# NVlabs/neuralrgbd

Measured on AMD Instinct MI355X. Metric: depth frames/sec @256x192x64cand, 5-view window; warp-kernel HBM GB/s vs peak, higher is better.
Workload: dtype f32; 1 GPU; plane-sweep grid 256x192x64cand (image 1024x768); config_id=B, depth_candidates=64, views=5, streams_per_gpu=1, streams_total=1, parallelism=replicas x1 (independent video streams)

## Files before the change

### include/nrgbd.h

```cpp
#ifndef NRGBD_H
#define NRGBD_H

#ifdef __cplusplus
extern "C" {
#endif

#define NRGBD_OK             0
#define NRGBD_E_NULL        -1
#define NRGBD_E_SHAPE       -2
#define NRGBD_E_ALIGN       -3
#define NRGBD_E_ARG         -4

#define NRGBD_DIST_L2        0
#define NRGBD_DIST_L1        1

#define NRGBD_MAX_D        256
#define NRGBD_MAX_V         16

#define NRGBD_INTERFACE_VERSION "0.10"
const char* nrgbd_version(void);
const char* nrgbd_strerror(int code);

int nrgbd_homography_terms(const float* K, const float* R, long r_view_stride, long r_row_stride,
                           const float* t, long t_view_stride, long t_elem_stride, float* KR, float* Kt,
// ... 130 lines not shown
int nrgbd_conv3d_wgrad_f32(const float* x, const float* gy, float* partial, float* dw,
                           int D, int H, int W, int Cin, void* stream);
int nrgbd_bn3d_finalize(const float* stats, int num_workgroups, long count,
                        const float* gamma, const float* beta, float eps, float momentum,
                        float* running_mean, float* running_var, float* scale_shift, unsigned int* collapse_count, long long* batches_tracked, void* stream);

int nrgbd_bn2d_partial_floats(int C);
int nrgbd_bn2d_train_act(const float* x, const float* gamma, const float* beta, float eps, int act,
                         const float* residual, float* y, float* partial, float* mean_var,
                         int N, int C, long HW, void* stream);
int nrgbd_avgpool8(const float* x, float* y, int NC, int H, int W, void* stream);
int nrgbd_avgpool_cl(const float* x, float* y, int N, int H, int W, int C, int k, void* stream);
int nrgbd_conv2d_few_f32(const float* x, int ldx, const float* w_packed, const float* bias, int out_lrelu, float* y, int ldy,
                         int ycoff, int N, int H, int W, int Cin, int Cout, void* stream);
int nrgbd_scatter_channels(const float* src, long stride_c, long stride_y, long stride_x, int C, int H, int W, float* dst,
                           int ldy, int coff, int n_rep, long rep_stride, void* stream);
int nrgbd_bias_act_nchw(float* x, const float* bias, float slope, int N, int C, long HW, void* stream);

int nrgbd_conv_wino_tiles(int N, int H, int W, int dilation);
int nrgbd_conv_wino_rnet_f32(const float* x, const float* w_wino, const float* bias, int out_lrelu, float* y,
                             int N, int H, int W, int Cin, int Cout, void* stream);
int nrgbd_conv_wino_rnet_ex_f32(const float* x, const float* w_wino, const float* bias, int out_lrelu, float* y,
                                int N, int H, int W, int Cin, int Cout, int ldy, int ycoff, int cout_valid, void* stream);
int nrgbd_conv_wino_pack(const float* w, float* w_wino, int Cin, int Cout, int kd, int transposed, void* stream);
int nrgbd_bn_finalize_cm(const float* stats, int rows, int C, long count, const float* gamma, const float* beta, float eps,
                         float momentum, float* running_mean, float* running_var, float* scale_shift, unsigned int* collapse_count,
                         long long* batches_tracked, void* stream);
int nrgbd_conv_wino_f32(const float* x, const float* x_ss, int x_relu, const float* res, const float* res_ss,
                        int res_relu, float* materialized, const float* w_wino, float* y, float* stats,
                        int N, int H, int W, int Cin, int Cout, int kd, int dilation, void* stream);

int nrgbd_conv_wino_dw_pack(const float* w, float* w_wino, int Cin, int Cout, int transposed, void* stream);
int nrgbd_conv_wino_dw_f32(const float* x, const float* x_ss, int x_relu, const float* res, const float* res_ss,
                           int res_relu, float* materialized, const float* w_wino, float* y, float* stats,
                           int N, int H, int W, int Cin, int Cout, void* stream);
int nrgbd_conv_wino_dw_workgroups(int N, int H, int W, int Cout);
int nrgbd_conv_wino_dw4_pack(const float* w, float* w_wino, int Cin, int Cout, int transposed, void* stream);
int nrgbd_conv_wino_dw4_workspace(int N, int H, int W, int Cout, size_t* bytes);
int nrgbd_conv_wino_dw4_f32(const float* x, const float* x_ss, int x_relu, float x_unit, const float* w_wino, float* y, float* stats,
                            void* workspace, size_t workspace_bytes, int N, int H, int W, int Cin, int Cout, void* stream);
int nrgbd_conv_wino_dw_unit_f32(const float* x, const float* x_ss, float x_unit, const float* w_wino, float* y, float* stats,
                                int N, int H, int W, int Cin, int Cout, void* stream);

int nrgbd_conv2d_rnet_f32(const float* x, const float* w_packed, const float* bias, int out_lrelu, float* y,
                          int ldy, int ycoff, int cout_valid, int mode, int pa, int pb,
                          int N, int H, int W, int Cin, int Cout, void* stream);
// ... 168 lines not shown
```

### neuralrgbd_amd/_lib.py

```python
import ctypes
import os

_HERE = os.path.dirname(os.path.abspath(__file__))
LIB_PATH = os.path.join(_HERE, "csrc", "libnrgbd_hip.so")

_c = ctypes
_P = _c.c_void_p
_F = _c.c_float
_I = _c.c_int
_L = _c.c_long
_D = _c.c_double
_Z = _c.c_size_t

GATHER_MAX_V = 6
DEPTH_MAX_THRESHOLDS = 512
DEPTH_EVAL_MAX_SETS = 8
DGF_TILE = (16, 64)
TSDF_EXTRACT_VOXELS = 1024
TSDF_SCAN_PASS = 1024
TSDF_RAYCAST_MAX_STEPS = 65536
TSDF_RAYCAST_TILE = 16
TSDF_RAYCAST_MAX_SIDE = 16384
ICP_MAX_WG = 256
ICP_RECORD_BYTES = 240
# ... 36 lines not shown
    "nrgbd_logsoftmax_d": (_I, [_P, _P, _F, _P, _I, _L, _P]),
    "nrgbd_depth_regress": (_I, [_P, _P, _P, _P, _I, _L, _P]),
    "nrgbd_export_depth_u16": (_I, [_P, _P, _F, _F, _P, _P, _P, _P, _I, _L, _P]),
    "nrgbd_depth_regress_rows": (_I, [_P, _P, _P, _P, _I, _L, _P]),
    "nrgbd_export_depth_u16_rows": (_I, [_P, _P, _F, _F, _P, _P, _P, _P, _I, _L, _P]),
    "nrgbd_warp_depth_fwd": (_I, [_P, _P, _P, _P, _P, _P, _P, _I, _I, _I, _I, _P]),
    "nrgbd_warp_depth_bwd_workgroups": (_I, [_I, _I]),
    "nrgbd_warp_depth_bwd": (_I, [_P, _P, _P, _P, _P, _P, _P, _P, _P, _P, _I, _I, _I, _I, _P]),
    "nrgbd_lba_pyramid": (_I, [_P, _I, _I, _I, _P, _I, _P, _P]),
    "nrgbd_lba_workgroups": (_I, [_I, _I]),
    "nrgbd_lba_grad": (_I, [_P, _P, _P, _P, _P, _P, _P, _P, _I, _I, _I, _P]),
    "nrgbd_lba_update": (_I, [_P, _I, _P, _P, _P, _I, _I, _I, _I, _I, _I, _I, _D, _I, _I, _P]),
    "nrgbd_conv3d_workgroups": (_I, [_I, _I, _I]),
    "nrgbd_conv3d_pack_weights": (_I, [_P, _P, _I, _P]),
    "nrgbd_conv3d_3x3x3_f32": (_I, [_P, _P, _I, _P, _P, _I, _P, _P, _P, _P, _I, _I, _I, _I, _I, _P]),
    "nrgbd_conv3d_3x3x3_cout1_f32": (_I, [_P, _P, _I, _P, _P, _I, _P, _P, _I, _I, _I, _I, _P]),
    "nrgbd_conv3d_cout1_bwd_workgroups": (_I, [_I, _I, _I, _I]),
    "nrgbd_conv3d_cout1_dgrad_f32": (_I, [_P, _P, _P, _I, _I, _I, _P]),
    "nrgbd_conv3d_cout1_wgrad_workspace": (_I, [_I, _I, _I, _P]),
    "nrgbd_conv3d_cout1_wgrad_f32": (_I, [_P, _P, _P, _P, _Z, _I, _I, _I, _P]),
    "nrgbd_conv_wino_tiles": (_I, [_I, _I, _I, _I]),
    "nrgbd_conv_wino_rnet_f32": (_I, [_P, _P, _P, _I, _P, _I, _I, _I, _I, _I, _P]),
    "nrgbd_conv_wino_rnet_ex_f32": (_I, [_P, _P, _P, _I, _P, _I, _I, _I, _I, _I, _I, _I, _I, _P]),
    "nrgbd_conv_wino_pack": (_I, [_P, _P, _I, _I, _I, _I, _P]),
    "nrgbd_bn_finalize_cm": (_I, [_P, _I, _I, _L, _P, _P, _F, _F, _P, _P, _P, _P, _P, _P]),
    "nrgbd_conv_wino_f32": (_I, [_P, _P, _I, _P, _P, _I, _P, _P, _P, _P, _I, _I, _I, _I, _I, _I, _I, _P]),
    "nrgbd_conv_wino_dw_pack": (_I, [_P, _P, _I, _I, _I, _P]),
    "nrgbd_conv_wino_dw_f32": (_I, [_P, _P, _I, _P, _P, _I, _P, _P, _P, _P, _I, _I, _I, _I, _I, _P]),
    "nrgbd_conv_wino_dw_workgroups": (_I, [_I, _I, _I, _I]),
    "nrgbd_conv_wino_dw_unit_f32": (_I, [_P, _P, _F, _P, _P, _P, _I, _I, _I, _I, _I, _P]),
    "nrgbd_conv_wino_dw4_pack": (_I, [_P, _P, _I, _I, _I, _P]),
    "nrgbd_conv_wino_dw4_workspace": (_I, [_I, _I, _I, _I, _P]),
    "nrgbd_conv_wino_dw4_f32": (_I, [_P, _P, _I, _F, _P, _P, _P, _P, _c.c_size_t, _I, _I, _I, _I, _I, _P]),
    "nrgbd_conv3d_wgrad_workgroups": (_I, []),
    "nrgbd_conv3d_wgrad_ranges": (_I, []),
    "nrgbd_conv3d_wgrad_f32": (_I, [_P, _P, _P, _P, _I, _I, _I, _I, _P]),
    "nrgbd_bn3d_finalize": (_I, [_P, _I, _L, _P, _P, _F, _F, _P, _P, _P, _P, _P, _P]),
    "nrgbd_bn2d_partial_floats": (_I, [_I]),
    "nrgbd_bn2d_train_act": (_I, [_P, _P, _P, _F, _I, _P, _P, _P, _P, _I, _I, _L, _P]),
    "nrgbd_avgpool8": (_I, [_P, _P, _I, _I, _I, _P]),
    "nrgbd_conv2d_few_f32": (_I, [_P, _I, _P, _P, _I, _P, _I, _I, _I, _I, _I, _I, _I, _P]),
    "nrgbd_avgpool_cl": (_I, [_P, _P, _I, _I, _I, _I, _I, _P]),
    "nrgbd_scatter_channels": (_I, [_P, _L, _L, _L, _I, _I, _I, _P, _I, _I, _I, _L, _P]),
    "nrgbd_bias_act_nchw": (_I, [_P, _P, _F, _I, _I, _L, _P]),
    "nrgbd_conv2d_workgroups": (_I, [_I, _I, _I]),
    "nrgbd_conv2d_wgrad_workgroups": (_I, [_I, _I, _I, _I, _I]),
# ... 96 lines not shown
```

### neuralrgbd_amd/csrc/wino_pc.hip

```cpp
#include "wino_pc.hpp"

namespace nrgbd {

namespace {

struct PcLane {
    int kq, jj;
    int msel, cwv;
    int a0, a1;
    unsigned ldy, lane_yoff;
};
template <bool HALF> using PcAcc = f32x4[16][HALF ? 1 : 2];

template <int DIL, int EPI, bool HALF>
__device__ __forceinline__ PcLane pc_lane(const WinoPcArgs& a, int lane, int wv) {
    PcLane c;
    c.kq = lane >> 4; c.jj = lane & 15;
    c.msel = HALF ? (wv >> 1) : 0;
    c.cwv = HALF ? (wv & 1) : wv;
    c.a0 = pc_slot(0, 16 * c.msel + c.jj, c.kq); c.a1 = pc_slot(0, 16 + c.jj, c.kq);
    c.ldy = (EPI == 1 && a.ldy) ? (unsigned)a.ldy : (unsigned)a.Cout;
    c.lane_yoff = (unsigned)c.jj + (unsigned)((DIL * 2 * (c.kq >> 1)) * a.W + 8 * (c.kq & 1) * DIL) * c.ldy;
    return c;
}
// ... 147 lines not shown
    s1 += __shfl_xor(s1, 16, 64); s2 += __shfl_xor(s2, 16, 64);
    s1 += __shfl_xor(s1, 32, 64); s2 += __shfl_xor(s2, 32, 64);
    if (c.kq == 0) {
        const int srow = HALF ? 2 * tl.row + c.msel : tl.row;
        a.stats[(size_t)co * a.rows + srow] = s1;
        a.stats[(size_t)(a.Cout + co) * a.rows + srow] = s2;
    }
}

template <int DIL, int EPI, bool HALF>
__device__ __forceinline__ void pc_epilogue(const PcAcc<HALF>& acc, const WinoPcArgs& a, const PcTile& tl, const PcLane& c) {
    const int co = tl.cg * 64 + c.cwv * 16 + c.jj;
    float* ybase = a.y + (((size_t)tl.n * a.H + tl.y0 + tl.py) * a.W + tl.x0 + tl.px) * c.ldy + (EPI == 1 ? a.ycoff : 0) + tl.cg * 64 + c.cwv * 16;
    const bool cok = EPI != 1 || a.cout_valid == 0 || co < a.cout_valid;
    const bool inside = tl.y0 + tl.py + DIL * (kPcTH - 1) < a.H && tl.x0 + tl.px + DIL * (kPcTW - 1) < a.W;
    float s1 = 0.f, s2 = 0.f;
    float bval = 0.f;
    if constexpr (EPI == 1) bval = a.bias ? a.bias[co] : 0.f;
    if (inside) pc_epilogue_interior<DIL, EPI, HALF>(acc, a, c, ybase, cok, bval, s1, s2);
    else pc_epilogue_edge<DIL, EPI, HALF>(acc, a, tl, c, ybase, cok, bval, s1, s2);
    if (a.stats) pc_store_stats<HALF>(a, tl, c, co, s1, s2);
}

struct PcItems {
    int id0, w4;
    int wr_off[kPcNPF];
    int rdR0, rdR1, rdR2;
    float sg, m1;
    int vslot;
    __device__ __forceinline__ int item_id(int u) const { return id0 + 64 * u; }
    __device__ __forceinline__ int row(int u) const { return (item_id(u) >> 2) / 18; }
    __device__ __forceinline__ int cp(int u) const { const int pi = item_id(u) >> 2; return pi - (pi / 18) * 18; }
    __device__ __forceinline__ int col(int u) const { const int c = cp(u); return c < 9 ? 2 * c : 2 * c - 17; }
};

__device__ __forceinline__ PcItems pc_items(int pw, int lane) {
    PcItems p;
    p.id0 = 192 * pw + lane;
    p.w4 = lane & 3;
#pragma unroll
    for (int u = 0; u < kPcNPF; ++u) {
        const int item = p.item_id(u), e = (item - kPcShItems) >> 2;
        p.wr_off[u] = item < kPcShItems ? (p.row(u) * kPcRawW + p.cp(u)) * kCB + p.w4 * 4
                                        : ((e >> 1) * kPcRawW + 18 + (e & 1)) * kCB + p.w4 * 4;
    }
    const int tword = lane & 3, thalf = (lane >> 4) & 1, txl = ((lane >> 5) << 2) | ((lane >> 2) & 3);
// ... 49 lines not shown
            r.rs[1] = *reinterpret_cast<const f32x4*>(P.ssl + 2 * a.Cin + 2 * (cb * kCB + w4 * 4) + 4);
        }
    }
    const int tz = nx ? P.tn.n : P.tl.n;
    const int z = KD == 3 ? min(max(tz + kd - 1, 0), a.N - 1) : 0;
    const size_t base = ((size_t)z * P.plane + (size_t)(cb * kCB)) * sizeof(float);
    const __amdgpu_buffer_rsrc_t xb = pc_rsrc(reinterpret_cast<const char*>(a.x) + base);
    const __amdgpu_buffer_rsrc_t rb = pc_rsrc(reinterpret_cast<const char*>(RES ? a.res : a.x) + base);
#pragma unroll
    for (int u = 0; u < kPcNPF; ++u) {
        const unsigned o = nx ? P.nxt.off[u] : P.cur.off[u];
        r.pre[u] = pc_bload(xb, o);
        if constexpr (RES) r.prer[u] = pc_bload(rb, o);
    }
}

template <int KD, bool RES, int EPI, bool MAT, bool INTERIOR>
__device__ __forceinline__ void pc_activate_publish(const WinoPcArgs& a, const PcProd& P, const PcRegs<RES>& r, float* raw, int cb, int kd, int z) {
    const f32x2 sc01 = r.ss[0].lo, sh01 = r.ss[0].hi, sc23 = r.ss[1].lo, sh23 = r.ss[1].hi;
    const f32x2 rc01 = r.rs[0].lo, rh01 = r.rs[0].hi, rc23 = r.rs[1].lo, rh23 = r.rs[1].hi;
    const bool wmat = MAT && (KD != 3 || kd == 1) && P.tl.cg == 0;
    constexpr int NU = kPcNPF;
    f32x2 lo[NU], hi[NU];
    if constexpr (EPI == 1) {
#pragma unroll
        for (int i = 0; i < NU; ++i) { lo[i] = r.pre[i].lo; hi[i] = r.pre[i].hi; }
    } else {
#pragma unroll
        for (int i = 0; i < NU; ++i) {
            lo[i] = __builtin_elementwise_fma(r.pre[i].lo, sc01, sh01);
            hi[i] = __builtin_elementwise_fma(r.pre[i].hi, sc23, sh23);
        }
    }
    __builtin_amdgcn_sched_barrier(0);
    if (EPI == 0 && a.x_relu) {
#pragma unroll
        for (int i = 0; i < NU; ++i) { lo[i].x = relu1(lo[i].x); lo[i].y = relu1(lo[i].y); hi[i].x = relu1(hi[i].x); hi[i].y = relu1(hi[i].y); }
    }
    __builtin_amdgcn_sched_barrier(0);
    if constexpr (RES) {
        f32x2 ql[NU], qh[NU];
#pragma unroll
        for (int i = 0; i < NU; ++i) {
            ql[i] = __builtin_elementwise_fma(r.prer[i].lo, rc01, rh01);
            qh[i] = __builtin_elementwise_fma(r.prer[i].hi, rc23, rh23);
        }
        __builtin_amdgcn_sched_barrier(0);
// ... 77 lines not shown
}

template <int KD, int DIL, bool RES, bool ODD = false, int EPI = 0, bool MAT = false, bool HALF = false>
__global__ __launch_bounds__(512) void conv_wino_pc_kernel(const WinoPcArgs a) {
    extern __shared__ __attribute__((aligned(16))) float lds[];
    float* Vb = lds;
    float* rawb = lds + kPcNBuf * kPcV;
    float* ssl = rawb + kPcStrips;

    const int tid = threadIdx.x, lane = tid & 63;
    const int wave = __builtin_amdgcn_readfirstlane(tid >> 6);
    const int wv = wave & 3;
    const int NS = (a.Cin / kCB) * KD;

    int first, step, end;
    pc_tile_share(a.ntiles, first, step, end);
    if (first >= end) return;
    const int count = (end - first + step - 1) / step;
    if constexpr (EPI == 0) {
        pc_load_ss_table<true>(ssl, a.Cin, a.x_ss, RES ? a.res_ss : nullptr, 1.f);
        __syncthreads();
    }

    if (wave >= 4) {
        const PcLane c = pc_lane<DIL, EPI, HALF>(a, lane, wv);
        PcAcc<HALF> acc;
        const f32x4* wbase = reinterpret_cast<const f32x4*>(a.wp) + c.cwv * 64 + lane;
        const size_t wgroup = (size_t)NS * 16 * 256;
        PcTile tl = pc_decode<KD, DIL>(first, a);
        const f32x4* wt = wbase + (size_t)tl.cg * wgroup;
        f32x4 Bn[kPcNB], An[4][2];
        pc_prime_weights<HALF>(Bn, wt);
        __syncthreads();
        __syncthreads();
        __syncthreads();
        pc_prime_a<HALF>(An, Vb, c);
        int buf = 0;
        for (int it = 0; it < count; ++it) {
            const int tnext = first + (it + 1 < count ? it + 1 : it) * step;
            const PcTile tn = pc_decode<KD, DIL>(tnext, a);
            const f32x4* wt_next = wbase + (size_t)tn.cg * wgroup;
            for (int s = 0; s < NS; ++s) {
                const float* Vc = Vb + buf * kPcV;
                const int nbuf = buf == kPcNBuf - 1 ? 0 : buf + 1;
                const float* Vn = Vb + nbuf * kPcV;
                const f32x4* wcur = wt + (size_t)s * (16 * 256);
// ... 86 lines not shown
    }
    const long idx = (long)blockIdx.x * 256 + threadIdx.x;
    if (idx >= total) return;
    long t = idx;
    const int e = t & 3; t >>= 2;
    const int j = t & 15; t >>= 4;
    const int kq = t & 3; t >>= 2;
    const int wave = t & 3; t >>= 2;
    const int xi = t & 15; t >>= 4;
    const int kd = (int)(t % KD); t /= KD;
    const int ncb = Cin / kCB;
    const int cb = (int)(t % ncb);
    const int cg = (int)(t / ncb);
    const int co = cg * 64 + 16 * wave + j, ci = cb * kCB + 4 * kq + e;
    const float* g = transposed ? w + (((size_t)ci * Cout + co) * KD + (KD - 1 - kd)) * 9 : w + (((size_t)co * Cin + ci) * KD + kd) * 9;
    const double G[4][3] = {{1.0, 0.0, 0.0}, {0.5, 0.5, 0.5}, {0.5, -0.5, 0.5}, {0.0, 0.0, 1.0}};
    const int a = xi >> 2, b = xi & 3;
    double u = 0.0;
#pragma unroll
    for (int ky = 0; ky < 3; ++ky)
#pragma unroll
        for (int kx = 0; kx < 3; ++kx) u += G[a][ky] * (double)g[transposed ? (2 - ky) * 3 + (2 - kx) : ky * 3 + kx] * G[b][kx];
    wp[idx] = (float)u;
}

static int pc_workgroups(long ntiles, int* nwg) {
    int dev = 0, ncu = 0;
    hipError_t e = hipGetDevice(&dev);
    if (e == hipSuccess) e = hipDeviceGetAttribute(&ncu, hipDeviceAttributeMultiprocessorCount, dev);
    if (e != hipSuccess) return (int)e;
    if (ncu <= 0) return NRGBD_E_ARG;
    *nwg = ntiles < ncu ? (int)ntiles : ncu;
    return NRGBD_OK;
}

struct PcLaunch { int nwg; size_t lds; int lds_attr; hipStream_t stream; };

template <int KD, int DIL, bool RES, bool ODD = false, int EPI = 0, bool MAT = false, bool HALF = false>
static hipError_t pc_launch(const PcLaunch& L, const WinoPcArgs& a) {
    const hipError_t e = set_max_dynamic_lds(reinterpret_cast<const void*>(&conv_wino_pc_kernel<KD, DIL, RES, ODD, EPI, MAT, HALF>), L.lds_attr);
    if (e != hipSuccess) return e;
    hipLaunchKernelGGL((conv_wino_pc_kernel<KD, DIL, RES, ODD, EPI, MAT, HALF>), dim3(L.nwg), dim3(512), L.lds, L.stream, a);
    return hipSuccess;
}

template <int KD, int DIL, bool HALF>
// ... 83 lines not shown
    if (cout_valid < 0 || cout_valid > Cout || ycoff < 0 || (ldy != 0 && ldy < ycoff + (cout_valid ? cout_valid : Cout))) return NRGBD_E_ARG;
    if ((long)N * H * W * (ldy ? ldy : Cout) >= (1L << 32)) return NRGBD_E_SHAPE;
    const int rows = nrgbd_conv_wino_tiles(N, H, W, 1);
    const long nt = (long)rows * (half ? 1 : Cout / 64);
    if (nt >= (1L << 30)) return NRGBD_E_SHAPE;
    WinoPcArgs a{x, nullptr, nullptr, nullptr, nullptr, w_wino, y, nullptr, 0, 0, N, H, W, Cin, Cout, (int)nt, half ? 2 * rows : rows,
                 bias, out_lrelu, ldy, ycoff, cout_valid};
    int nwg = 0;
    const int rc = pc_workgroups(nt, &nwg);
    if (rc != NRGBD_OK) return rc;
    const size_t lds = (size_t)(kPcNBuf * kPcV + kPcStrips) * sizeof(float);
    const PcLaunch L{nwg, lds, (int)lds, (hipStream_t)stream};
    const bool odd = ((Cin / kCB) & 1) != 0;
    hipError_t e;
    if (odd && half) e = pc_launch<1, 1, false, true, 1, false, true>(L, a);
    else if (odd) e = pc_launch<1, 1, false, true, 1, false, false>(L, a);
    else if (half) e = pc_launch<1, 1, false, false, 1, false, true>(L, a);
    else e = pc_launch<1, 1, false, false, 1, false, false>(L, a);
    if (e != hipSuccess) return (int)e;
    NRGBD_CHECK_LAUNCH();
    return NRGBD_OK;
}

extern "C" int nrgbd_conv_wino_rnet_f32(const float* x, const float* w_wino, const float* bias, int out_lrelu, float* y, int N,
                                        int H, int W, int Cin, int Cout, void* stream) {
    return nrgbd_conv_wino_rnet_ex_f32(x, w_wino, bias, out_lrelu, y, N, H, W, Cin, Cout, 0, 0, 0, stream);
}
```

### neuralrgbd_amd/nets.py

```python
import math

import numpy as np
import torch
import torch.nn as nn
import torch.nn.functional as F


def _conv_bn2d(cin, cout, k, stride, pad, dilation, track=False):
    p = dilation if dilation > 1 else pad
    return nn.Sequential(
        nn.Conv2d(cin, cout, k, stride=stride, padding=p, dilation=dilation, bias=False),
        nn.BatchNorm2d(cout, track_running_stats=track),
    )


def _conv_bn3d(cin, cout):
    return nn.Sequential(nn.Conv3d(cin, cout, 3, stride=1, padding=1, bias=False), nn.BatchNorm3d(cout))


def _conv_lrelu(cin, cout):
    return nn.Sequential(nn.Conv2d(cin, cout, 3, stride=1, padding=1, bias=True), nn.LeakyReLU())


def _deconv_lrelu(cin, cout):
# ... 568 lines not shown
                og = np.ogrid[:n, :n]
                bil = (1 - abs(og[0] - center) / factor) * (1 - abs(og[1] - center) / factor)
                m.weight.data.copy_(torch.from_numpy(bil))

    def _widths(self):
        D = self.conv2_2.out_channels
        C0 = self.conv0[0].in_channels - D
        C1 = self.conv1[0].in_channels - D
        C2 = self.conv2[0].in_channels - D
        ok = 1 <= D <= 128 and (C0, C1, C2) == (64, 32, 3) and self.trans_conv0[0].out_channels == D \
            and self.trans_conv1[0].out_channels == D and self.conv2_1[0].out_channels == D
        return (D, 64 if D <= 64 else 128, C0, C1, C2) if ok else None

    def _levels(self):
        wd = self._widths()
        if wd is not None:
            return ((wd[0], wd[1]),) * 3
        D = self.conv0[0].in_channels - 64
        D0, D1 = self.trans_conv0[0].out_channels, self.conv2_2.out_channels
        ok = D in (32, 64) and (D0, D1) == (2 * D, 4 * D) and self.conv1[0].in_channels == D0 + 32 \
            and self.trans_conv1[0].out_channels == D1 and self.conv2[0].in_channels == D1 + 3 and self.conv2_1[0].out_channels == D1
        return ((D, 64), (D0, D0), (D1, D1)) if ok else None

    _FEATS = (64, 32, 3)

    def mfma_ok(self, dpv):
        return dpv.is_cuda and not torch.is_grad_enabled() and dpv.dtype == torch.float32

    def _embedded(self):
        lv = self._levels()
        C0, C1, C2 = self._FEATS
        mods = {"conv0": self.conv0[0], "conv0_1": self.conv0_1[0], "trans_conv0": self.trans_conv0[0], "conv1": self.conv1[0],
                "conv1_1": self.conv1_1[0], "trans_conv1": self.trans_conv1[0], "conv2": self.conv2[0], "conv2_1": self.conv2_1[0],
                "conv2_2": self.conv2_2}
        if all(d == dp for d, dp in lv):
            return {k: (m.weight.detach(), m.bias.detach()) for k, m in mods.items()}
        dev = self.conv2_2.weight.device
        cat = lambda l, C: (torch.cat((torch.arange(lv[l][0], device=dev), lv[l][1] + torch.arange(C, device=dev))), lv[l][1] + C)
        plain = lambda l: (torch.arange(lv[l][0], device=dev), lv[l][1])
        io = {"conv0": cat(0, C0) + cat(0, C0), "conv0_1": cat(0, C0) + cat(0, C0), "trans_conv0": cat(0, C0) + plain(1),
              "conv1": cat(1, C1) + cat(1, C1), "conv1_1": cat(1, C1) + cat(1, C1), "trans_conv1": cat(1, C1) + plain(2),
              "conv2": cat(2, C2) + cat(2, C2), "conv2_1": cat(2, C2) + plain(2), "conv2_2": plain(2) + plain(2)}
        out = {}
        for k, m in mods.items():
            in_idx, cin_p, out_idx, cout_p = io[k]
            w, b = m.weight.detach(), m.bias.detach()
# ... 11 lines not shown

    def _rnet_packed(self):
        from . import ops
        cache = self.__dict__.setdefault("_pk_cache", {})
        key = tuple((p.data_ptr(), p._version) for p in self.parameters())
        if cache.get("key") == key:
            return cache["val"]
        pad16 = lambda c: (c + 15) // 16 * 16
        pad32 = pad16
        emb = self._embedded()

        def deconv(name):
            w, b = emb[name]
            res = {}
            for pa in (0, 1):
                for pb in (0, 1):
                    ky = [3, 1] if pa == 0 else [2, 0]
                    kx = [3, 1] if pb == 0 else [2, 0]
                    wph = w[:, :, ky][:, :, :, kx].permute(1, 0, 2, 3)
                    res[(pa, pb)] = [(ops.conv_pack_weights(wph[c0:c0 + 64].contiguous()), b[c0:c0 + 64].contiguous(), 64, c0, 64)
                                     for c0 in range(0, w.shape[1], 64)]
            res["all"] = [(torch.cat([res[(pa, pb)][i][0] for pa in (0, 1) for pb in (0, 1)]),) + res[(0, 0)][i][1:]
                          for i in range(len(res[(0, 0)]))]
            return res

        def wino(name):
            w, b = emb[name]
            cin_p, cout_p = pad32(w.shape[1]), (w.shape[0] + 63) // 64 * 64
            wp = w.new_zeros(cout_p, cin_p, 3, 3)
            wp[:w.shape[0], :w.shape[1]] = w
            bp = b.new_zeros(cout_p)
            bp[:w.shape[0]] = b
            extra = w.shape[0] % 64
            if 0 < extra <= 4 and w.shape[0] > 64:
                full = w.shape[0] - extra
                few = wp[full:full + extra].reshape(extra, cin_p // 16, 16, 9).permute(1, 3, 0, 2).contiguous()
                return (ops.conv_wino_pack(wp[:full].contiguous()), bp[:full].contiguous(), full, full,
                        ("few", few, bp[full:full + extra].contiguous(), extra, full))
            if 0 < extra <= 32 and w.shape[0] > 64:
                full = w.shape[0] - extra
                tail = wp.new_zeros(64, cin_p, 3, 3)
                tail[:extra] = wp[full:full + extra]
                return (ops.conv_wino_pack(wp[:full].contiguous()), bp[:full].contiguous(), full, full,
                        (ops.conv_wino_pack(tail), bp[full:full + 32].contiguous(), 32, extra, full))
            return (ops.conv_wino_pack(wp.contiguous()), bp.contiguous(), cout_p, w.shape[0])

# ... 28 lines not shown
                dpv_log = torch.cat(list(dpv_log), dim=0)
            return self.forward(torch.exp(dpv_log), img_features)
        from . import ops
        lv = self._levels()
        if lv is None:
            raise _no_kernel("this R-Net (image-feature widths other than 64 / 32 / 3, more than 128 candidates, or candidate "
                             "up-sampling from other than 32 or 64 candidates)")
        (D, Dp), (_, Dp1), (Dl, Dpl) = lv
        quarter, half, full = img_features
        if isinstance(dpv_log, (list, tuple)):
            vols = [v[i:i + 1] for v in dpv_log for i in range(v.shape[0])]
        else:
            vols = [dpv_log[i:i + 1] for i in range(dpv_log.shape[0])]
        n = len(vols)
        _, _, h, w = vols[0].shape
        if n > 2:
            return torch.cat([self.forward_log(vols[i:i + 2], img_features).clone() for i in range(0, n, 2)], dim=0)
        if tuple(quarter.shape) != (1, 64, h, w) or tuple(half.shape) != (1, 32, 2 * h, 2 * w) or tuple(full.shape) != (1, 3, 4 * h, 4 * w):
            raise ValueError("forward_log: features of ONE image at 1/4, 1/2 and full resolution ([1,64,h,w], [1,32,2h,2w], [1,3,4h,4w]) expected")
        dev = first.device
        pk, buf = self._rnet_packed(), self._rnet_buffers(n, h, w, dev)

        def deconv(x, layer, out):
            for wp, bias, wdt, c0, valid in layer:
                ops.conv2d_rnet(x, wp, wdt, bias=bias, out=out, ldy=out.shape[-1], ycoff=c0, cout_valid=valid, mode=3)
            return out

        def conv_w(x, name, out=None, lrelu=True):
            wt = pk[name + "_w"]
            out = ops.conv_wino_rnet(x, wt[0], wt[2], bias=wt[1], lrelu=lrelu, out=out, cout_valid=wt[3])
            if len(wt) > 4:
                t = wt[4]
                if t[0] == "few":
                    ops.conv2d_few(x, t[1], bias=t[2], lrelu=lrelu, out=out, ycoff=t[4])
                else:
                    ops.conv_wino_rnet(x, t[0], t[2], bias=t[1], lrelu=lrelu, out=out, ycoff=t[4], cout_valid=t[3])
            return out

        if D != Dp:
            for b in range(n):
                buf["dpv"][b, :D].copy_(vols[b][0])
            vols = [buf["dpv"][b:b + 1] for b in range(n)]
        q_cl = quarter.permute(0, 2, 3, 1)
        x = buf["x0"]
        for b in range(n):
            if q_cl.is_contiguous():
                ops.rnet_pack(vols[b][0].contiguous(), q_cl[0], feat_planar=False, out=x[b:b + 1])
            else:
                ops.rnet_pack(vols[b][0].contiguous(), quarter[0].contiguous(), feat_planar=True, out=x[b:b + 1])
        x = conv_w(conv_w(x, "conv0", buf["a0"]), "conv0_1", buf["b0"])
        c1 = buf["c1"]
        deconv(x, pk["t0"]["all"], c1)
        ops.scatter_channels(half[0], c1, Dp1)
        x = conv_w(conv_w(c1, "conv1", buf["a1"]), "conv1_1", buf["b1"])
        c2 = buf["c2"]
        deconv(x, pk["t1"]["all"], c2)
        ops.scatter_channels(full[0], c2, Dpl)
        x = conv_w(conv_w(c2, "conv2", buf["g2"]), "conv2_1", buf["h2"])
        y = ops.logsoftmax_rows(conv_w(x, "conv2_2", None, lrelu=False)).permute(0, 3, 1, 2)
        return y if Dl == Dpl else y[:, :Dl]

    def forward(self, dpv_raw, img_features):
        quarter, half, full = img_features
        from .autograd import LogSoftmaxCL, cat_cl, conv2d_module, conv_transpose2d_module, padded_in_width

        def cl(m, x):
            return conv2d_module(m[0], x, act_slope=0.01)

        def tl(m, x):
            return conv_transpose2d_module(m[0], x, act_slope=0.01)
        x = cl(self.conv0_1, cl(self.conv0, cat_cl([dpv_raw, quarter], padded_in_width(self.conv0[0]))))
        x = tl(self.trans_conv0, x)
        x = cl(self.conv1_1, cl(self.conv1, cat_cl([x, half], padded_in_width(self.conv1[0]))))
        x = tl(self.trans_conv1, x)
        x = conv2d_module(self.conv2[0], cat_cl([x, full], padded_in_width(self.conv2[0])), keep_width=True, act_slope=0.01)
        x = conv2d_module(self.conv2_2, cl(self.conv2_1, x))
        if LogSoftmaxCL.supported(x) and x.permute(0, 2, 3, 1).is_contiguous():
            return LogSoftmaxCL.apply(x)
        return torch.log_softmax(x, dim=1)
# ... 70 lines not shown
```

### neuralrgbd_amd/ops.py

```python
import ctypes
import typing

import numpy as np
import torch

from . import _lib

DIST = {"L2": 0, "L1": 1}
GENERATION = {None: 0, "auto": 0, "gather": 1, "lds": 2, "quad": 3}


def _need(t, name, shape=None, strided=False):
    if not isinstance(t, torch.Tensor):
        raise TypeError("%s must be a torch.Tensor" % name)
    if not t.is_cuda:
        raise _lib.NrgbdError("%s is on %s: the plane-sweep path runs on the GPU only "
                              "(no CPU fallback)" % (name, t.device))
    if t.dtype != torch.float32:
        raise TypeError("%s must be float32, got %s" % (name, t.dtype))
    if shape is not None and tuple(t.shape) != tuple(shape):
        raise ValueError("%s has shape %s, expected %s" % (name, tuple(t.shape), tuple(shape)))
    return t if (strided or t.is_contiguous()) else t.contiguous()


# ... 874 lines not shown
                raise ValueError("bn_small_stats: %s must be contiguous (it is updated in place)" % name)
        _nbt_ptr(nbts[i], xs[i])
    keep = (ptrs(xs), (ctypes.c_long * n)(*[x.numel() // C for x in xs]), ptrs(gammas), ptrs(betas), (ctypes.c_float * n)(*eps),
            (ctypes.c_float * n)(*momentum), ptrs(rms), ptrs(rvs), ptrs(nbts), ptrs(ss))
    with torch.cuda.device(dev):
        rc = _lib.load().nrgbd_bn_small_stats(n, *[ctypes.cast(a, ctypes.c_void_p) for a in keep[:2]], int(C),
                                          *[ctypes.cast(a, ctypes.c_void_p) for a in keep[2:]], _stream(xs[0]))
    _lib.check(rc, "nrgbd_bn_small_stats")
    return ss


def conv_wino_rnet(x, w_wino, cout, bias=None, lrelu=True, out=None, ycoff=0, cout_valid=None):
    x = _need(x, "x")
    N, H, W, Cin = x.shape
    valid = int(cout if cout_valid is None else cout_valid)
    if out is None:
        out = torch.empty((N, H, W, valid), dtype=torch.float32, device=x.device)
    elif tuple(out.shape[:3]) != (N, H, W) or not out.is_contiguous() or out.shape[3] < ycoff + valid:
        raise ValueError("conv_wino_rnet: out must be a contiguous [N,H,W,>= ycoff + cout_valid] tensor")
    with torch.cuda.device(x.device):
        rc = _lib.load().nrgbd_conv_wino_rnet_ex_f32(_p(x), _p(w_wino), _p(bias), int(bool(lrelu)), _p(out), N, H, W, Cin, int(cout),
                                                      int(out.shape[3]), int(ycoff), valid, _stream(x))
    _lib.check(rc, "nrgbd_conv_wino_rnet_ex_f32")
    return out


def conv2d_few(x, w_few, bias=None, lrelu=True, out=None, ycoff=0):
    x = _need(x, "x")
    w_few = _need(w_few, "w_few")
    N, H, W, ldx = x.shape
    nblk, taps, cout, lanes = w_few.shape
    if taps != 9 or lanes != 16 or not 1 <= cout <= 4 or nblk * 16 > ldx:
        raise ValueError("conv2d_few: w_few %s for an input of %d channels" % (tuple(w_few.shape), ldx))
    if out is None:
        out = torch.empty((N, H, W, cout), dtype=torch.float32, device=x.device)
    elif tuple(out.shape[:3]) != (N, H, W) or not out.is_contiguous() or out.shape[3] < ycoff + cout:
        raise ValueError("conv2d_few: out must be a contiguous [N,H,W,>= ycoff + Cout] tensor")
    with torch.cuda.device(x.device):
        rc = _lib.load().nrgbd_conv2d_few_f32(_p(x), int(ldx), _p(w_few), _p(bias), int(bool(lrelu)), _p(out), int(out.shape[3]), int(ycoff),
                                               N, H, W, nblk * 16, cout, _stream(x))
    _lib.check(rc, "nrgbd_conv2d_few_f32")
    return out


def bn_cl_supported(rows, C):
    return rows > 0 and 4 <= C <= 1024 and C % 4 == 0 and 256 % (C // 4) == 0
# ... 1063 lines not shown
```

Measured before the change: 31.68 frames/s.

## Run refinement-net transposed convs through a phase-split Winograd kernel with masked points

```diff
diff --git a/include/nrgbd.h b/include/nrgbd.h
--- a/include/nrgbd.h
+++ b/include/nrgbd.h
@@ -176,6 +176,9 @@
                              int N, int H, int W, int Cin, int Cout, void* stream);
 int nrgbd_conv_wino_rnet_ex_f32(const float* x, const float* w_wino, const float* bias, int out_lrelu, float* y,
                                 int N, int H, int W, int Cin, int Cout, int ldy, int ycoff, int cout_valid, void* stream);
+int nrgbd_conv_wino_rnet_deconv_f32(const float* x, const float* w_masked, const float* bias, int out_lrelu, float* y,
+                                    int N, int H, int W, int Cin, int Cout, int ldy, int ycoff, int cout_valid, void* stream);
+int nrgbd_conv_wino_rnet_deconv_pack(const float* w_wino, float* w_masked, int Cin, void* stream);
 int nrgbd_conv_wino_pack(const float* w, float* w_wino, int Cin, int Cout, int kd, int transposed, void* stream);
 int nrgbd_bn_finalize_cm(const float* stats, int rows, int C, long count, const float* gamma, const float* beta, float eps,
                          float momentum, float* running_mean, float* running_var, float* scale_shift, unsigned int* collapse_count,
diff --git a/neuralrgbd_amd/_lib.py b/neuralrgbd_amd/_lib.py
--- a/neuralrgbd_amd/_lib.py
+++ b/neuralrgbd_amd/_lib.py
@@ -82,6 +82,8 @@
     "nrgbd_conv_wino_tiles": (_I, [_I, _I, _I, _I]),
     "nrgbd_conv_wino_rnet_f32": (_I, [_P, _P, _P, _I, _P, _I, _I, _I, _I, _I, _P]),
     "nrgbd_conv_wino_rnet_ex_f32": (_I, [_P, _P, _P, _I, _P, _I, _I, _I, _I, _I, _I, _I, _I, _P]),
+    "nrgbd_conv_wino_rnet_deconv_f32": (_I, [_P, _P, _P, _I, _P, _I, _I, _I, _I, _I, _I, _I, _I, _P]),
+    "nrgbd_conv_wino_rnet_deconv_pack": (_I, [_P, _P, _I, _P]),
     "nrgbd_conv_wino_pack": (_I, [_P, _P, _I, _I, _I, _I, _P]),
     "nrgbd_bn_finalize_cm": (_I, [_P, _I, _I, _L, _P, _P, _F, _F, _P, _P, _P, _P, _P, _P]),
     "nrgbd_conv_wino_f32": (_I, [_P, _P, _I, _P, _P, _I, _P, _P, _P, _P, _I, _I, _I, _I, _I, _I, _I, _P]),
diff --git a/neuralrgbd_amd/csrc/wino_pc.hip b/neuralrgbd_amd/csrc/wino_pc.hip
--- a/neuralrgbd_amd/csrc/wino_pc.hip
+++ b/neuralrgbd_amd/csrc/wino_pc.hip
@@ -193,6 +193,185 @@
     if (a.stats) pc_store_stats<HALF>(a, tl, c, co, s1, s2);
 }
 
+constexpr int kPcDcPts = 9;
+template <int PH> __device__ constexpr int pc_dc_xi(int p) { return 4 * (p / 3 + (PH >> 1)) + p % 3 + (PH & 1); }
+template <int PH> __device__ constexpr bool pc_dc_live(int xi) {
+    return (xi >> 2) >= (PH >> 1) && (xi >> 2) < (PH >> 1) + 3 && (xi & 3) >= (PH & 1) && (xi & 3) < (PH & 1) + 3;
+}
+__device__ __forceinline__ int pc_dc_first(int ph) { return (4 * (ph >> 1) + (ph & 1)) * (kPcTiles * kCB); }
+
+__device__ __forceinline__ PcLane pc_dc_lane(const WinoPcArgs& a, int lane, int wv) {
+    PcLane c;
+    c.kq = lane >> 4; c.jj = lane & 15;
+    c.msel = 0; c.cwv = wv;
+    c.a0 = pc_slot(0, c.jj, c.kq); c.a1 = pc_slot(0, 16 + c.jj, c.kq);
+    c.ldy = 2u * (unsigned)a.ldy;
+    c.lane_yoff = (unsigned)c.jj + (unsigned)((2 * (c.kq >> 1)) * (2 * a.W) + 8 * (c.kq & 1)) * c.ldy;
+    return c;
+}
+
+template <int PH, bool FIRST>
+__device__ __forceinline__ void pc_dc_stage(PcAcc<false>& acc, f32x4 (&An)[3][2], f32x4 (&Bn)[kPcDcPts], const float* Vc, const float* Vn, int nx0,
+                                            const f32x4* wcur, const f32x4* wnx, const PcLane& c) {
+    const int a0 = c.a0, a1 = c.a1;
+    const f32x4 zero4 = {0.f, 0.f, 0.f, 0.f};
+#pragma unroll
+    for (int p = 0; p < kPcDcPts; ++p) {
+        const int xi = pc_dc_xi<PH>(p), cur = p % 3, nxt = (p + 2) % 3;
+        if (p + 2 < kPcDcPts) {
+            An[nxt][0] = *reinterpret_cast<const f32x4*>(Vc + a0 + pc_dc_xi<PH>(p + 2) * (kPcTiles * kCB));
+            An[nxt][1] = *reinterpret_cast<const f32x4*>(Vc + a1 + pc_dc_xi<PH>(p + 2) * (kPcTiles * kCB));
+        } else {
+            An[nxt][0] = *reinterpret_cast<const f32x4*>(Vn + a0 + nx0 + (p + 2 - kPcDcPts) * (kPcTiles * kCB));
+            An[nxt][1] = *reinterpret_cast<const f32x4*>(Vn + a1 + nx0 + (p + 2 - kPcDcPts) * (kPcTiles * kCB));
+        }
+#pragma unroll
+        for (int e = 0; e < 4; ++e) {
+            acc[xi][0] = __builtin_amdgcn_mfma_f32_16x16x4f32(An[cur][0][e], Bn[p][e], FIRST && e == 0 ? zero4 : acc[xi][0], 0, 0, 0);
+            acc[xi][1] = __builtin_amdgcn_mfma_f32_16x16x4f32(An[cur][1][e], Bn[p][e], FIRST && e == 0 ? zero4 : acc[xi][1], 0, 0, 0);
+            if (e == kPcWPos) Bn[(p + kPcBD) % kPcDcPts] = p + kPcBD < kPcDcPts ? wcur[(p + kPcBD) * 256] : wnx[(p + kPcBD - kPcDcPts) * 256];
+            __builtin_amdgcn_sched_barrier(0);
+        }
+    }
+}
+
+template <int PH>
+__device__ __forceinline__ void pc_dc_epilogue_interior(const PcAcc<false>& acc, const WinoPcArgs& a, const PcLane& c, float* ybase, bool cok, float bval) {
+    const unsigned ldy = c.ldy, lane_yoff = c.lane_yoff;
+    const size_t W2 = 2 * (size_t)a.W;
+    float neg1 = -1.f;
+    asm volatile("" : "+v"(neg1));
+    const f32x2 n1 = {neg1, neg1};
+    const f32x2 bias2 = {bval, bval};
+    const f32x2 z2 = {0.f, 0.f};
+#pragma unroll
+    for (int m = 0; m < 2; ++m) {
+#pragma unroll
+        for (int rp = 0; rp < 2; ++rp) {
+            f32x2 tr[2][4];
+#pragma unroll
+            for (int xx = 0; xx < 4; ++xx) {
+                const f32x2 m0 = !pc_dc_live<PH>(0 + xx) ? z2 : rp ? acc[0 + xx][m].hi : acc[0 + xx][m].lo;
+                const f32x2 m1 = !pc_dc_live<PH>(4 + xx) ? z2 : rp ? acc[4 + xx][m].hi : acc[4 + xx][m].lo;
+                const f32x2 m2 = !pc_dc_live<PH>(8 + xx) ? z2 : rp ? acc[8 + xx][m].hi : acc[8 + xx][m].lo;
+                const f32x2 m3 = !pc_dc_live<PH>(12 + xx) ? z2 : rp ? acc[12 + xx][m].hi : acc[12 + xx][m].lo;
+                tr[0][xx] = (m0 + m1) + m2;
+                tr[1][xx] = __builtin_elementwise_fma(m3, n1, __builtin_elementwise_fma(m2, n1, m1));
+            }
+#pragma unroll
+            for (int aa = 0; aa < 2; ++aa) {
+                f32x2 o0 = (tr[aa][0] + tr[aa][1]) + tr[aa][2];
+                f32x2 o1 = __builtin_elementwise_fma(tr[aa][3], n1, __builtin_elementwise_fma(tr[aa][2], n1, tr[aa][1]));
+                o0 = o0 + bias2; o1 = o1 + bias2;
+                if (a.out_lrelu) {
+                    const f32x2 sl = {0.01f, 0.01f};
+                    o0 = __builtin_elementwise_max(o0, o0 * sl); o1 = __builtin_elementwise_max(o1, o1 * sl);
+                }
+                float* oa = ybase + ((size_t)(4 * m + aa) * W2 + (size_t)(2 * (2 * rp))) * ldy;
+                float* ob = ybase + ((size_t)(4 * m + aa) * W2 + (size_t)(2 * (2 * rp + 1))) * ldy;
+                if (cok) {
+                    oa[lane_yoff] = o0.x; oa[lane_yoff + ldy] = o1.x;
+                    ob[lane_yoff] = o0.y; ob[lane_yoff + ldy] = o1.y;
+                }
+            }
+        }
+    }
+}
+
+template <int PH>
+__device__ __forceinline__ void pc_dc_epilogue_edge(const PcAcc<false>& acc, const WinoPcArgs& a, const PcTile& tl, const PcLane& c, float* ybase,
+                                                    bool cok, float bval) {
+    const unsigned ldy = c.ldy, lane_yoff = c.lane_yoff;
+    const size_t W2 = 2 * (size_t)a.W;
+#pragma unroll
+    for (int m = 0; m < 2; ++m) {
+#pragma unroll
+        for (int r = 0; r < 4; ++r) {
+            float tr[2][4];
+#pragma unroll
+            for (int xx = 0; xx < 4; ++xx) {
+                const float m0 = pc_dc_live<PH>(0 + xx) ? acc[0 + xx][m][r] : 0.f, m1 = pc_dc_live<PH>(4 + xx) ? acc[4 + xx][m][r] : 0.f;
+                const float m2 = pc_dc_live<PH>(8 + xx) ? acc[8 + xx][m][r] : 0.f, m3 = pc_dc_live<PH>(12 + xx) ? acc[12 + xx][m][r] : 0.f;
+                tr[0][xx] = (m0 + m1) + m2;
+                tr[1][xx] = (m1 - m2) - m3;
+            }
+#pragma unroll
+            for (int aa = 0; aa < 2; ++aa) {
+                float o0 = (tr[aa][0] + tr[aa][1]) + tr[aa][2];
+                float o1 = (tr[aa][1] - tr[aa][2]) - tr[aa][3];
+                o0 += bval; o1 += bval;
+                if (a.out_lrelu) { o0 = fmaxf(o0, 0.01f * o0); o1 = fmaxf(o1, 0.01f * o1); }
+                float* o = ybase + ((size_t)(4 * m + aa) * W2 + (size_t)(2 * r)) * ldy;
+                const int tile = 16 * m + 4 * c.kq + r;
+                const int gy = tl.y0 + 2 * (tile >> 3) + aa, gx = tl.x0 + 2 * (tile & 7);
+                if (gy < a.H && cok) {
+                    if (gx < a.W) o[lane_yoff] = o0;
+                    if (gx + 1 < a.W) o[lane_yoff + ldy] = o1;
+                }
+            }
+        }
+    }
+}
+
+template <int PH>
+__device__ __forceinline__ void pc_dc_tile(const WinoPcArgs& a, const PcTile& tl, int nph, int NS, f32x4 (&An)[3][2], f32x4 (&Bn)[kPcDcPts],
+                                           const float* Vb, int& buf, const f32x4* wt, const f32x4* wt_next, const PcLane& c) {
+    PcAcc<false> acc;
+    for (int s = 0; s < NS; ++s) {
+        const float* Vc = Vb + buf * kPcV;
+        const int nbuf = buf == kPcNBuf - 1 ? 0 : buf + 1;
+        const float* Vn = Vb + nbuf * kPcV;
+        const f32x4* wcur = wt + (size_t)s * (kPcDcPts * 256);
+        const bool last = s + 1 == NS;
+        const f32x4* wnx = last ? wt_next : wcur + kPcDcPts * 256;
+        const int nx0 = pc_dc_first(last ? nph : PH);
+        if (s == 0) pc_dc_stage<PH, true>(acc, An, Bn, Vc, Vn, nx0, wcur, wnx, c);
+        else pc_dc_stage<PH, false>(acc, An, Bn, Vc, Vn, nx0, wcur, wnx, c);
+        __syncthreads();
+        buf = nbuf;
+    }
+    const int co = c.cwv * 16 + c.jj;
+    float* ybase = a.y + (((size_t)tl.n * (2 * a.H) + 2 * tl.y0 + (PH >> 1)) * (2 * (size_t)a.W) + 2 * tl.x0 + (PH & 1)) * a.ldy + a.ycoff + c.cwv * 16;
+    const bool cok = co < a.cout_valid;
+    const bool inside = tl.y0 + (kPcTH - 1) < a.H && tl.x0 + (kPcTW - 1) < a.W;
+    const float bval = a.bias ? a.bias[co] : 0.f;
+    if (inside) pc_dc_epilogue_interior<PH>(acc, a, c, ybase, cok, bval);
+    else pc_dc_epilogue_edge<PH>(acc, a, tl, c, ybase, cok, bval);
+}
+
+__device__ __forceinline__ void pc_dc_consumer(const WinoPcArgs& a, const float* Vb, int NS, int first, int step, int count, int lane, int wv) {
+    const PcLane c = pc_dc_lane(a, lane, wv);
+    const f32x4* wbase = reinterpret_cast<const f32x4*>(a.wp) + wv * 64 + lane;
+    const size_t wgroup = (size_t)NS * kPcDcPts * 256;
+    PcTile tl = pc_decode<1, 1>(first, a);
+    const f32x4* wt = wbase + (size_t)tl.cg * wgroup;
+    f32x4 Bn[kPcDcPts], An[3][2];
+#pragma unroll
+    for (int b = 0; b < kPcBD; ++b) Bn[b] = wt[b * 256];
+    __syncthreads();
+    __syncthreads();
+    __syncthreads();
+#pragma unroll
+    for (int i = 0; i < 2; ++i) {
+        An[i][0] = *reinterpret_cast<const f32x4*>(Vb + c.a0 + pc_dc_first(tl.cg) + i * kPcTiles * kCB);
+        An[i][1] = *reinterpret_cast<const f32x4*>(Vb + c.a1 + pc_dc_first(tl.cg) + i * kPcTiles * kCB);
+    }
+    int buf = 0;
+    for (int it = 0; it < count; ++it) {
+        const int tnext = first + (it + 1 < count ? it + 1 : it) * step;
+        const PcTile tn = pc_decode<1, 1>(tnext, a);
+        const f32x4* wt_next = wbase + (size_t)tn.cg * wgroup;
+        switch (__builtin_amdgcn_readfirstlane(tl.cg)) {
+            case 0: pc_dc_tile<0>(a, tl, tn.cg, NS, An, Bn, Vb, buf, wt, wt_next, c); break;
+            case 1: pc_dc_tile<1>(a, tl, tn.cg, NS, An, Bn, Vb, buf, wt, wt_next, c); break;
+            case 2: pc_dc_tile<2>(a, tl, tn.cg, NS, An, Bn, Vb, buf, wt, wt_next, c); break;
+            default: pc_dc_tile<3>(a, tl, tn.cg, NS, An, Bn, Vb, buf, wt, wt_next, c); break;
+        }
+        tl = tn;
+        wt = wt_next;
+    }
+}
+
 struct PcItems {
     int id0, w4;
     int wr_off[kPcNPF];
@@ -288,7 +467,7 @@
     const bool wmat = MAT && (KD != 3 || kd == 1) && P.tl.cg == 0;
     constexpr int NU = kPcNPF;
     f32x2 lo[NU], hi[NU];
-    if constexpr (EPI == 1) {
+    if constexpr (EPI >= 1) {
 #pragma unroll
         for (int i = 0; i < NU; ++i) { lo[i] = r.pre[i].lo; hi[i] = r.pre[i].hi; }
     } else {
@@ -412,6 +591,9 @@
         __syncthreads();
     }
 
+    if constexpr (EPI == 2) {
+        if (wave >= 4) { pc_dc_consumer(a, Vb, NS, first, step, count, lane, wv); return; }
+    }
     if (wave >= 4) {
         const PcLane c = pc_lane<DIL, EPI, HALF>(a, lane, wv);
         PcAcc<HALF> acc;
@@ -544,6 +726,19 @@
 #pragma unroll
         for (int kx = 0; kx < 3; ++kx) u += G[a][ky] * (double)g[transposed ? (2 - ky) * 3 + (2 - kx) : ky * 3 + kx] * G[b][kx];
     wp[idx] = (float)u;
+}
+
+__global__ __launch_bounds__(256) void conv_wino_deconv_pack_kernel(const f32x4* __restrict__ wp, f32x4* __restrict__ wm, int NS) {
+    const long total = 4L * NS * kPcDcPts * 256;
+    const long idx = (long)blockIdx.x * 256 + threadIdx.x;
+    if (idx >= total) return;
+    const int in = (int)(idx & 255);
+    long t = idx >> 8;
+    const int p = (int)(t % kPcDcPts); t /= kPcDcPts;
+    const int s = (int)(t % NS);
+    const int ph = (int)(t / NS);
+    const int xi = 4 * (p / 3 + (ph >> 1)) + p % 3 + (ph & 1);
+    wm[idx] = wp[(((long)ph * NS + s) * 16 + xi) * 256 + in];
 }
 
 static int pc_workgroups(long ntiles, int* nwg) {
@@ -673,6 +868,47 @@
     return NRGBD_OK;
 }
 
+extern "C" int nrgbd_conv_wino_rnet_deconv_pack(const float* w_wino, float* w_masked, int Cin, void* stream) {
+    using namespace nrgbd;
+    if (!w_wino || !w_masked) return NRGBD_E_NULL;
+    if (Cin <= 0 || Cin % kCB) return NRGBD_E_SHAPE;
+    if ((reinterpret_cast<uintptr_t>(w_wino) | reinterpret_cast<uintptr_t>(w_masked)) & 15) return NRGBD_E_ALIGN;
+    const int NS = Cin / kCB;
+    const long total = 4L * NS * kPcDcPts * 256;
+    hipLaunchKernelGGL(conv_wino_deconv_pack_kernel, dim3((unsigned)((total + 255) / 256)), dim3(256), 0, (hipStream_t)stream,
+                       reinterpret_cast<const f32x4*>(w_wino), reinterpret_cast<f32x4*>(w_masked), NS);
+    NRGBD_CHECK_LAUNCH();
+    return NRGBD_OK;
+}
+
+extern "C" int nrgbd_conv_wino_rnet_deconv_f32(const float* x, const float* w_masked, const float* bias, int out_lrelu, float* y, int N,
+                                               int H, int W, int Cin, int Cout, int ldy, int ycoff, int cout_valid, void* stream) {
+    using namespace nrgbd;
+    if (!x || !w_masked || !y) return NRGBD_E_NULL;
+    if (N <= 0 || H <= 0 || W <= 0 || Cin < 32 || Cin % kCB || ((Cin / kCB) & 1) || Cout != 64) return NRGBD_E_SHAPE;
+    if ((long)N * H * W * Cin >= (1L << 30)) return NRGBD_E_SHAPE;
+    if (ldy == 0) ldy = Cout;
+    if (cout_valid == 0) cout_valid = Cout;
+    if (cout_valid < 0 || cout_valid > Cout || ycoff < 0 || ldy < ycoff + cout_valid) return NRGBD_E_ARG;
+    if (4L * N * H * W * ldy >= (1L << 31)) return NRGBD_E_SHAPE;
+    if ((reinterpret_cast<uintptr_t>(x) | reinterpret_cast<uintptr_t>(w_masked)) & 15) return NRGBD_E_ALIGN;
+    if ((reinterpret_cast<uintptr_t>(y) | reinterpret_cast<uintptr_t>(bias)) & 3) return NRGBD_E_ALIGN;
+    const int rows = nrgbd_conv_wino_tiles(N, H, W, 1);
+    const long nt = (long)rows * 4;
+    if (nt >= (1L << 30)) return NRGBD_E_SHAPE;
+    WinoPcArgs a{x, nullptr, nullptr, nullptr, nullptr, w_masked, y, nullptr, 0, 0, N, H, W, Cin, 4 * Cout, (int)nt, rows,
+                 bias, out_lrelu, ldy, ycoff, cout_valid};
+    int nwg = 0;
+    const int rc = pc_workgroups(nt, &nwg);
+    if (rc != NRGBD_OK) return rc;
+    const size_t lds = (size_t)(kPcNBuf * kPcV + kPcStrips) * sizeof(float);
+    const PcLaunch L{nwg, lds, (int)lds, (hipStream_t)stream};
+    const hipError_t e = pc_launch<1, 1, false, false, 2, false, false>(L, a);
+    if (e != hipSuccess) return (int)e;
+    NRGBD_CHECK_LAUNCH();
+    return NRGBD_OK;
+}
+
 extern "C" int nrgbd_conv_wino_rnet_f32(const float* x, const float* w_wino, const float* bias, int out_lrelu, float* y, int N,
                                         int H, int W, int Cin, int Cout, void* stream) {
     return nrgbd_conv_wino_rnet_ex_f32(x, w_wino, bias, out_lrelu, y, N, H, W, Cin, Cout, 0, 0, 0, stream);
diff --git a/neuralrgbd_amd/nets.py b/neuralrgbd_amd/nets.py
--- a/neuralrgbd_amd/nets.py
+++ b/neuralrgbd_amd/nets.py
@@ -614,6 +614,7 @@
             and self.trans_conv1[0].out_channels == D1 and self.conv2[0].in_channels == D1 + 3 and self.conv2_1[0].out_channels == D1
         return ((D, 64), (D0, D0), (D1, D1)) if ok else None
 
+    deconv_kernels = ("wino", "direct")
     _FEATS = (64, 32, 3)
 
     def mfma_ok(self, dpv):
@@ -671,6 +672,13 @@
                                      for c0 in range(0, w.shape[1], 64)]
             res["all"] = [(torch.cat([res[(pa, pb)][i][0] for pa in (0, 1) for pb in (0, 1)]),) + res[(0, 0)][i][1:]
                           for i in range(len(res[(0, 0)]))]
+            cin_p = pad16(w.shape[0])
+            res["wino"] = None
+            if cin_p % 32 == 0 and w.shape[1] % 64 == 0:
+                wi = w.new_zeros((cin_p,) + tuple(w.shape[1:]))
+                wi[:w.shape[0]] = w
+                res["wino"] = [(ops.conv_wino_rnet_deconv_pack(ops.conv_wino_pack(ops.deconv_phase_weights(wi[:, c0:c0 + 64])), cin_p),
+                                b[c0:c0 + 64].contiguous(), 64, c0, 64) for c0 in range(0, w.shape[1], 64)]
             return res
 
         def wino(name):
@@ -745,8 +753,13 @@
         pk, buf = self._rnet_packed(), self._rnet_buffers(n, h, w, dev)
 
         def deconv(x, layer, out):
-            for wp, bias, wdt, c0, valid in layer:
-                ops.conv2d_rnet(x, wp, wdt, bias=bias, out=out, ldy=out.shape[-1], ycoff=c0, cout_valid=valid, mode=3)
+            wino = self.deconv_kernels[0] == "wino" and layer["wino"] is not None \
+                and ops.conv_wino_rnet_deconv_supported(x.shape[0], x.shape[1], x.shape[2], x.shape[3], out.shape[-1])
+            for wp, bias, wdt, c0, valid in layer["wino" if wino else "all"]:
+                if wino:
+                    ops.conv_wino_rnet_deconv(x, wp, out, bias=bias, ycoff=c0, cout_valid=valid)
+                else:
+                    ops.conv2d_rnet(x, wp, wdt, bias=bias, out=out, ldy=out.shape[-1], ycoff=c0, cout_valid=valid, mode=3)
             return out
 
         def conv_w(x, name, out=None, lrelu=True):
@@ -773,11 +786,11 @@
                 ops.rnet_pack(vols[b][0].contiguous(), quarter[0].contiguous(), feat_planar=True, out=x[b:b + 1])
         x = conv_w(conv_w(x, "conv0", buf["a0"]), "conv0_1", buf["b0"])
         c1 = buf["c1"]
-        deconv(x, pk["t0"]["all"], c1)
+        deconv(x, pk["t0"], c1)
         ops.scatter_channels(half[0], c1, Dp1)
         x = conv_w(conv_w(c1, "conv1", buf["a1"]), "conv1_1", buf["b1"])
         c2 = buf["c2"]
-        deconv(x, pk["t1"]["all"], c2)
+        deconv(x, pk["t1"], c2)
         ops.scatter_channels(full[0], c2, Dpl)
         x = conv_w(conv_w(c2, "conv2", buf["g2"]), "conv2_1", buf["h2"])
         y = ops.logsoftmax_rows(conv_w(x, "conv2_2", None, lrelu=False)).permute(0, 3, 1, 2)
diff --git a/neuralrgbd_amd/ops.py b/neuralrgbd_amd/ops.py
--- a/neuralrgbd_amd/ops.py
+++ b/neuralrgbd_amd/ops.py
@@ -920,6 +920,48 @@
         rc = _lib.load().nrgbd_conv_wino_rnet_ex_f32(_p(x), _p(w_wino), _p(bias), int(bool(lrelu)), _p(out), N, H, W, Cin, int(cout),
                                                       int(out.shape[3]), int(ycoff), valid, _stream(x))
     _lib.check(rc, "nrgbd_conv_wino_rnet_ex_f32")
+    return out
+
+
+def deconv_phase_weights(w):
+    from .autograd import _tap_select
+    cin, cout = w.shape[:2]
+    idx, msk = _tap_select("t2", w.device)
+    w4 = w.detach().permute(1, 0, 2, 3).reshape(cout, cin, 16).index_select(2, idx) * msk
+    return w4.reshape(cout, cin, 4, 9).permute(2, 0, 1, 3).reshape(4 * cout, cin, 3, 3).contiguous()
+
+
+def deconv_live_points(phase):
+    a, b = phase >> 1, phase & 1
+    return [4 * (r + a) + c + b for r in range(3) for c in range(3)]
+
+
+def conv_wino_rnet_deconv_pack(w_wino, Cin):
+    w_wino = _need(w_wino, "w_wino")
+    if w_wino.numel() != 256 * Cin * 16:
+        raise ValueError("conv_wino_rnet_deconv_pack: a 256-column stream of %d input channels expected" % Cin)
+    wm = torch.empty(4 * (Cin // 16) * 9 * 1024, dtype=torch.float32, device=w_wino.device)
+    with torch.cuda.device(w_wino.device):
+        rc = _lib.load().nrgbd_conv_wino_rnet_deconv_pack(_p(w_wino), _p(wm), int(Cin), _stream(w_wino))
+    _lib.check(rc, "nrgbd_conv_wino_rnet_deconv_pack")
+    return wm
+
+
+def conv_wino_rnet_deconv_supported(N, H, W, Cin, ldy):
+    return Cin >= 32 and Cin % 32 == 0 and N * H * W * Cin < (1 << 30) and 4 * N * H * W * ldy < (1 << 31)
+
+
+def conv_wino_rnet_deconv(x, w_masked, out, bias=None, lrelu=True, ycoff=0, cout_valid=64):
+    x = _need(x, "x")
+    N, H, W, Cin = x.shape
+    if tuple(out.shape[:3]) != (N, 2 * H, 2 * W) or not out.is_contiguous() or out.shape[3] < ycoff + cout_valid:
+        raise ValueError("conv_wino_rnet_deconv: out must be a contiguous [N,2H,2W,>= ycoff + cout_valid] tensor")
+    if w_masked.numel() != 4 * (Cin // 16) * 9 * 1024:
+        raise ValueError("conv_wino_rnet_deconv: the masked stream does not belong to %d input channels" % Cin)
+    with torch.cuda.device(x.device):
+        rc = _lib.load().nrgbd_conv_wino_rnet_deconv_f32(_p(x), _p(w_masked), _p(bias), int(bool(lrelu)), _p(out), N, H, W, Cin, 64,
+                                                          int(out.shape[3]), int(ycoff), int(cout_valid), _stream(x))
+    _lib.check(rc, "nrgbd_conv_wino_rnet_deconv_f32")
     return out
 
 
```

Result: faster. 32.00 frames/s, median of 6 (+1.0%).
